# MeryylleA/Lunaris-Orion

Hardware: AMD Instinct MI355X
Metric: 128x128 sprites/sec, VAE training step (train_hybrid.py _process_batch), latent_dim=512 (higher is better)
Workload: dtype f16; 1 GPU; VAE-only training step (fwd+MSE/KL+bwd+clip+AdamW), per-GPU batch 64, latent_dim 512, teacher scalar 0 (--reward_scale 0 --quality_weight 0; the full hybrid step of BASELINE config 3 is the config3_full_hybrid object of a --full run at N=1), gradient_accumulation_steps 1, fp16 MFMA operands / fp32 accumulate, fp32 master weights; global_batch=64, latent_dim=512, parallelism=single, linear_weight_gradients=factored (never materialised)

## Files before the change

### include/lunaris_hip.h

```cpp
#ifndef LUNARIS_HIP_H
#define LUNARIS_HIP_H
#include <stddef.h>
#include <stdint.h>
#ifdef __cplusplus
extern "C" {
#endif

const char* lo_last_error(void);
int lo_version(void);

void lo_prof_enable(int on);
int lo_prof_count(void);
int lo_prof_get(int i, char* name, int name_cap, double* ms, double* flops, double* bytes);

enum {
  LO_KIND_CONV3_S1 = 0,
  LO_KIND_CONV3_S2 = 1,
  LO_KIND_CONVT4_S2 = 2,
  LO_KIND_CONV3_S1_DGRAD = 3,
  LO_KIND_CONV3_S2_DGRAD = 4,
  LO_KIND_CONVT4_S2_DGRAD = 5,
  LO_KIND_LINEAR = 6
};


size_t lo_packed_weight_elems_for(int kind, int B, int H, int W, int Cin, int Cout);
int lo_pack_weight_for(int kind, int B, int H, int W, int Cin, int Cout, const float* w, void* wp, void* stream);
int lo_conv_forward(int kind, int B, int H, int W, int Cin, int Cout, const void* in, const void* wp, const float* bias,
                    const void* add_src, void* out, float* gn_partial, int* mt_out, void* stream);
int lo_quantize_act_f8(const void* x16, void* x8, size_t n, void* stream);
int lo_pack_weight_f8_for(int kind, int B, int H, int W, int Cin, int Cout, const void* wp16, void* wp8, float* wscale, void* stream);
int lo_conv_forward_f8(int kind, int B, int H, int W, int Cin, int Cout, const void* in8, const void* wp8, const float* wscale,
                       const float* bias, const void* add_src, void* out, float* gn_partial, int* mt_out, void* stream);
int lo_conv3x3_fused_tap_forward(int B, int H, int W, int Cin, int Cout, int fp8, const void* in, const void* wp, const float* wscale,
                                 const float* bias, int leaky_relu, void* out, float* bn_partial, void* stream);
int lo_teacher_conv3x3_forward_f8(int B, int H, int W, int Cin, int Cout, const void* in8, const void* wp8, const float* wscale,
                                  const float* bias, int leaky_relu, void* out, float* bn_partial, int* rows_out, void* stream);
int lo_linear_splitk(int M, int K, int N, const void* x, const void* wp, const float* bias, float* slab, int nsplit,
                     float* out32, void* out16, void* stream);
size_t lo_wgrad_slab_bytes_for(int kind, int B, int H, int W, int Cin, int Cout);
int lo_conv_wgrad(int kind, int B, int H, int W, int Cin, int Cout, const void* x, const void* dy, float* slab,
                  float* grad, float scale, void* stream);

int lo_gn_mish_forward(const void* v, const float* gn_partial, int MT, const float* gamma, const float* beta,
                       const void* other, void* y, float* stats, int B, int HW, int C, int mode, void* stream);
int lo_gn_nchunk_for(int HW, int C);
int lo_gn_mish_backward(const void* dy, const void* v, const void* other, const float* stats, const float* gamma,
                        const float* beta, void* ds, void* dv, float* P1, float* P2, float* dgamma, float* dbeta,
                        float* dbias, int B, int HW, int C, int mode, float scale, void* stream);

int lo_first_conv_forward(const float* x, const float* w, const float* bias, void* v, float* gn_partial, int B, void* stream);
int lo_first_conv_wgrad_op(const float* x, const void* dv, float* partial , float* dw, int B, float scale, void* stream);
int lo_image_dgrad_op(const void* dy, int cout, int stride, const float* w, int B, float scale, float* dx, void* stream);
int lo_final_conv_forward(const void* a4, const float* w, const float* bias, const float* target, float* recon,
                          float* mse_partial, int B, void* stream);
int lo_final_conv_backward(const void* a4, const float* w, const float* recon, const float* target, const float* drecon,
                           const float* coef_dev, float gscale, void* da4, float* partial , float* dw,
                           float* db, int B, float scale, void* stream);

int lo_decode_sprites_u8(const void* u8_hwc, float* out_chw, int B, void* stream);

int lo_selfattn2d_forward(const float* x, const float* wq, const float* bq, const float* wk, const float* bk, const float* wv,
                          const float* bv, const float* gamma, float* q, float* k, float* v, float* out, int B, int C,
                          int N, void* stream);
size_t lo_selfattn2d_backward_scratch_elems(int B, int C, int N);
int lo_selfattn2d_backward(const float* x, const float* wq, const float* wk, const float* wv, const float* gamma,
                           const float* q, const float* k, const float* v, const float* dy, float* scratch, float* dx,
                           float* dwq, float* dbq, float* dwk, float* dbk, float* dwv, float* dbv, float* dgamma, int B,
                           int C, int N, void* stream);

int lo_clip_adamw_step(float* p, const float* g, float* m, float* v, size_t n, float max_norm, float lr, float beta1,
                       float beta2, float eps, float weight_decay, int step, float* scratch, void* stream);

int lo_clip_adamw_step_presummed(float* p, const float* g, float* m, float* v, size_t n, size_t presummed_begin, float max_norm,
                                 float lr, float beta1, float beta2, float eps, float weight_decay, int step, float* scratch,
                                 void* stream);

typedef struct LoVae LoVae;
int lo_vae_create(int batch, int latent_dim, LoVae** out);
#define LO_VAE_FP8_FWD 1u
int lo_vae_create_ex(int batch, int latent_dim, unsigned flags, LoVae** out);
void lo_vae_destroy(LoVae* h);
int lo_vae_set_gradnorm_scratch(LoVae* h, float* scratch);
int lo_gradnorm_early_range(const float* flat_grads, size_t begin, size_t end, float* scratch, void* stream);
int lo_vae_set_async_handover(LoVae* h, int on);
int lo_vae_wait_handover(LoVae* h, void* stream);
int lo_vae_gradnorm_presummed(const LoVae* h);
int lo_vae_num_params(const LoVae* h);
// ... 111 lines not shown
```

### lunaris_orion_amd/_lib.py

```python
from __future__ import annotations

import ctypes as C
import os

import torch

HERE = os.path.dirname(os.path.abspath(__file__))
LIB_PATH = os.path.join(HERE, "liblunaris_hip.so")

if not os.path.exists(LIB_PATH):
    raise ImportError(
        f"{LIB_PATH} not found: build it with `python -m lunaris_orion_amd.build` (hipcc, gfx950). "
        "There is no CPU or PyTorch fallback for the lunaris_orion_amd hot path."
    )

lib = C.CDLL(LIB_PATH, mode=C.RTLD_GLOBAL)

vp, f32p, i32, sz, u64, flt = C.c_void_p, C.c_void_p, C.c_int, C.c_size_t, C.c_uint64, C.c_float

SIGNATURES = {
    "lo_last_error": (C.c_char_p, []),
    "lo_version": (i32, []),
    "lo_prof_enable": (None, [i32]),
    "lo_prof_count": (i32, []),
    "lo_prof_get": (i32, [i32, C.c_char_p, i32, C.POINTER(C.c_double), C.POINTER(C.c_double), C.POINTER(C.c_double)]),
    "lo_packed_weight_elems_for": (sz, [i32] * 6),
    "lo_pack_weight_for": (i32, [i32] * 6 + [f32p, vp, vp]),
    "lo_conv_forward": (i32, [i32] * 6 + [vp, vp, f32p, vp, vp, f32p, C.POINTER(C.c_int), vp]),
    "lo_quantize_act_f8": (i32, [vp, vp, sz, vp]),
    "lo_pack_weight_f8_for": (i32, [i32] * 6 + [vp, vp, f32p, vp]),
    "lo_conv_forward_f8": (i32, [i32] * 6 + [vp, vp, f32p, f32p, vp, vp, f32p, C.POINTER(C.c_int), vp]),
    "lo_conv3x3_fused_tap_forward": (i32, [i32] * 6 + [vp, vp, f32p, f32p, i32, vp, f32p, vp]),
    "lo_teacher_conv3x3_forward_f8": (i32, [i32] * 5 + [vp, vp, f32p, f32p, i32, vp, f32p, C.POINTER(C.c_int), vp]),
    "lo_linear_splitk": (i32, [i32, i32, i32, vp, vp, f32p, f32p, i32, f32p, vp, vp]),
    "lo_wgrad_slab_bytes_for": (sz, [i32] * 6),
    "lo_conv_wgrad": (i32, [i32] * 6 + [vp, vp, f32p, f32p, flt, vp]),
    "lo_gn_mish_forward": (i32, [vp, f32p, i32, f32p, f32p, vp, vp, f32p, i32, i32, i32, i32, vp]),
    "lo_gn_nchunk_for": (i32, [i32, i32]),
    "lo_gn_mish_backward": (i32, [vp, vp, vp, f32p, f32p, f32p, vp, vp, f32p, f32p, f32p, f32p, f32p, i32, i32, i32, i32, flt, vp]),
    "lo_first_conv_forward": (i32, [f32p, f32p, f32p, vp, f32p, i32, vp]),
    "lo_first_conv_wgrad_op": (i32, [f32p, vp, f32p, f32p, i32, flt, vp]),
    "lo_image_dgrad_op": (i32, [vp, i32, i32, f32p, i32, flt, f32p, vp]),
    "lo_final_conv_forward": (i32, [vp, f32p, f32p, f32p, f32p, f32p, i32, vp]),
    "lo_final_conv_backward": (i32, [vp, f32p, f32p, f32p, f32p, f32p, flt, vp, f32p, f32p, f32p, i32, flt, vp]),
    "lo_decode_sprites_u8": (i32, [vp, f32p, i32, vp]),
    "lo_selfattn2d_forward": (i32, [f32p] * 12 + [i32, i32, i32, vp]),
    "lo_selfattn2d_backward_scratch_elems": (C.c_size_t, [i32, i32, i32]),
    "lo_selfattn2d_backward": (i32, [f32p] * 18 + [i32, i32, i32, vp]),
    "lo_clip_adamw_step": (i32, [f32p, f32p, f32p, f32p, sz, flt, flt, flt, flt, flt, flt, i32, f32p, vp]),
    "lo_teacher_create": (i32, [i32, i32, i32, i32, C.POINTER(C.c_void_p)]),
    "lo_teacher_create_ex": (i32, [i32, i32, i32, i32, C.c_uint, C.POINTER(C.c_void_p)]),
    "lo_teacher_destroy": (None, [vp]),
    "lo_teacher_num_tensors": (i32, [vp]),
    "lo_teacher_tensor_name": (C.c_char_p, [vp, i32]),
    "lo_teacher_tensor_numel": (sz, [vp, i32]),
    "lo_teacher_tensor_offset": (C.c_longlong, [vp, i32]),
    "lo_teacher_flat_elems": (sz, [vp]),
    "lo_teacher_workspace_bytes": (sz, [vp]),
    "lo_teacher_pack": (i32, [vp, f32p, vp, vp]),
    "lo_teacher_forward": (i32, [vp, f32p, f32p, vp, i32, flt, u64, f32p, f32p, f32p, f32p, f32p, vp]),
    "lo_teacher_last_path": (i32, [vp]),
    "lo_dropout_mask": (i32, [u64, i32, flt, sz, vp, vp]),
    "lo_teacher_grad_range": (i32, [vp, C.POINTER(C.c_size_t), C.POINTER(C.c_size_t)]),
    "lo_teacher_heads_backward": (i32, [vp, f32p, vp, f32p, flt, f32p, f32p, vp]),
    "lo_teacher_heads_saved": (i32, [vp, C.POINTER(C.c_size_t), C.POINTER(C.c_size_t)]),
    "lo_teacher_full_backward_bytes": (C.c_size_t, [vp]),
    "lo_teacher_full_backward_ex": (i32, [vp, f32p, f32p, vp, vp, f32p, f32p, f32p, f32p, f32p, f32p, flt, u64, flt, f32p, f32p, vp]),
    "lo_teacher_full_backward_dx": (i32, [vp, f32p, f32p, vp, vp, f32p, f32p, f32p, f32p, f32p, f32p, flt, u64, flt, f32p, f32p, f32p, vp]),
    "lo_teacher_forward_keep": (i32, [vp, f32p, f32p, vp, vp, flt, u64, f32p, f32p, f32p, f32p, f32p, vp]),
    "lo_teacher_full_backward": (i32, [vp, f32p, f32p, vp, vp, f32p, flt, flt, f32p, f32p, vp]),
    "lo_teacher_clip_adamw_full": (i32, [vp, f32p, f32p, f32p, f32p, flt, flt, flt, flt, flt, flt, i32, f32p, vp]),
    "lo_teacher_full_param_count": (i32, [vp, C.POINTER(C.c_size_t), C.POINTER(C.c_size_t)]),
    "lo_teacher_heads_backward_ex": (i32, [vp, f32p, f32p, f32p, f32p, f32p, f32p, f32p, flt, u64, f32p, f32p, vp]),
    "lo_hybrid_reward": (i32, [f32p, f32p, i32, flt, flt, flt, flt, flt, f32p, f32p, f32p, vp]),
    "lo_vae_create": (i32, [i32, i32, C.POINTER(C.c_void_p)]),
    "lo_vae_create_ex": (i32, [i32, i32, C.c_uint, C.POINTER(C.c_void_p)]),
# ... 79 lines not shown
```

### lunaris_orion_amd/csrc/lo_api.hip

```cpp
#include "lo_internal.h"
#include "lo_conv.h"
#include "lo_norm.h"
#include "../../include/lunaris_hip.h"
#include <stdio.h>
#include <string.h>
#include <stdlib.h>
#include <vector>


extern "C" const char* lo_last_error(void) { return lo_get_error(); }
extern "C" int lo_version(void) { return 1; }

extern "C" size_t lo_packed_weight_elems_for(int kind, int B, int H, int W, int Cin, int Cout) {
  LoGeom g;
  if (lo_make_geom(&g, kind, B, H, W, Cin, Cout) != LO_OK) return 0;
  return lo_packed_weight_elems(g);
}
extern "C" int lo_pack_weight_for(int kind, int B, int H, int W, int Cin, int Cout, const float* w, void* wp, void* stream) {
  LoGeom g;
  LO_TRY(lo_make_geom(&g, kind, B, H, W, Cin, Cout));
  return lo_pack_weight(w, (f16*)wp, g, S(stream));
}
extern "C" int lo_conv_forward(int kind, int B, int H, int W, int Cin, int Cout, const void* in, const void* wp,
                               const float* bias, const void* add_src, void* out, float* gn_partial, int* mt_out,
// ... 69 lines not shown
  LoGeom g;
  LO_REQUIRE(kind == LO_CONV3_S1 || kind == LO_CONV3_S2 || kind == LO_CONVT4_S2 || kind == LO_LINEAR,
             "lo_conv_wgrad: kind %d is not a forward op", kind);
  LO_TRY(lo_make_geom(&g, kind, B, H, W, Cin, Cout));
  return lo_wgrad_run(g, (const f16*)x, (const f16*)dy, slab, grad, scale, S(stream));
}
extern "C" int lo_gn_mish_forward(const void* v, const float* gn_partial, int MT, const float* gamma, const float* beta,
                                  const void* other, void* y, float* stats, int B, int HW, int C, int mode, void* stream) {
  return lo_gn_forward({(const f16*)v, stats, gamma, beta, B, HW, C},
                       {.partial = gn_partial, .MT = MT, .other = (const f16*)other, .mode = mode, .y = (f16*)y}, S(stream));
}
extern "C" int lo_gn_nchunk_for(int HW, int C) { return lo_gn_nchunk(HW, C); }
extern "C" int lo_gn_mish_backward(const void* dy, const void* v, const void* other, const float* stats, const float* gamma,
                                   const float* beta, void* ds, void* dv, float* P1, float* P2, float* dgamma, float* dbeta,
                                   float* dbias, int B, int HW, int C, int mode, float scale, void* stream) {
  return lo_gn_bwd({(const f16*)v, stats, gamma, beta, B, HW, C},
                   {.dy = (const f16*)dy, .other = (const f16*)other, .mode = mode, .ds = (f16*)ds, .dv = (f16*)dv, .P1 = P1, .P2 = P2},
                   dgamma, dbeta, dbias, scale, S(stream));
}
extern "C" int lo_first_conv_forward(const float* x, const float* w, const float* bias, void* v, float* gn_partial, int B,
                                     void* stream) {
  return lo_first_conv_fwd(x, w, bias, (f16*)v, gn_partial, B, S(stream));
}
extern "C" int lo_first_conv_wgrad_op(const float* x, const void* dv, float* partial, float* dw, int B, float scale, void* stream) {
  return lo_first_conv_wgrad(x, (const f16*)dv, partial, dw, B, scale, S(stream));
}
extern "C" int lo_image_dgrad_op(const void* dy, int cout, int stride, const float* w, int B, float scale, float* dx, void* stream) {
  return lo_image_dgrad((const f16*)dy, cout, stride, w, B, scale, dx, S(stream));
}
extern "C" int lo_final_conv_forward(const void* a4, const float* w, const float* bias, const float* target, float* recon,
                                     float* mse_partial, int B, void* stream) {
  return lo_final_conv_fwd((const f16*)a4, w, bias, target, recon, mse_partial, B, S(stream));
}
extern "C" int lo_final_conv_backward(const void* a4, const float* w, const float* recon, const float* target,
                                      const float* drecon, const float* coef_dev, float gscale, void* da4, float* partial,
                                      float* dw, float* db, int B, float scale, void* stream) {
  return lo_final_conv_bwd((const f16*)a4, w, recon, target, drecon, coef_dev, gscale, (f16*)da4, partial, dw, db, B, scale,
                           S(stream));
}
extern "C" int lo_clip_adamw_step(float* p, const float* g, float* m, float* v, size_t n, float max_norm, float lr,
                                  float beta1, float beta2, float eps, float weight_decay, int step, float* scratch,
                                  void* stream) {
  LO_TRY(lo_gradnorm(g, n, max_norm, scratch, scratch + 1024, S(stream)));
  return lo_adamw(p, g, m, v, n, scratch + 1024, lr, beta1, beta2, eps, weight_decay, step, S(stream));
}

extern "C" int lo_clip_adamw_step_presummed(float* p, const float* g, float* m, float* v, size_t n, size_t presummed_begin, float max_norm,
                                            float lr, float beta1, float beta2, float eps, float weight_decay, int step, float* scratch,
                                            void* stream) {
  LO_REQUIRE(p && g && m && v && scratch && presummed_begin <= n && presummed_begin % 4 == 0, "lo_clip_adamw_step_presummed: bad argument");
  LO_TRY(lo_gradnorm_split(g, presummed_begin, max_norm, scratch, scratch + 1024, S(stream)));
  return lo_adamw(p, g, m, v, n, scratch + 1024, lr, beta1, beta2, eps, weight_decay, step, S(stream));
}

extern "C" int lo_decode_sprites_u8(const void* u8_hwc, float* out_chw, int B, void* stream) {
  LO_REQUIRE(u8_hwc && out_chw && B > 0, "lo_decode_sprites_u8: bad argument");
  return lo_decode_sprites((const uint8_t*)u8_hwc, out_chw, B, S(stream));
}

extern "C" int lo_selfattn2d_forward(const float* x, const float* wq, const float* bq, const float* wk, const float* bk,
                                     const float* wv, const float* bv, const float* gamma, float* q, float* k, float* v,
                                     float* out, int B, int C, int N, void* stream) {
  LO_REQUIRE(x && wq && bq && wk && bk && wv && bv && gamma && q && k && v && out, "lo_selfattn2d_forward: null argument");
  return lo_selfattn2d_fwd(x, wq, bq, wk, bk, wv, bv, gamma, q, k, v, out, B, C, N, S(stream));
}

// ... 43 lines not shown
```

### lunaris_orion_amd/csrc/lo_edge.hip

```cpp
#include "lo_common.h"
#include <stdlib.h>

#define FC_W 128
#define FC_OW 64
#define FC_CO 64

__device__ __forceinline__ void fc_stage_rows(const float* __restrict__ x, float (*xs)[3][FC_W + 2], int n, int oy, int tid) {
  for (int i = tid; i < 3 * 3 * (FC_W + 2); i += 256) {
    int col = i % (FC_W + 2);
    int r = (i / (FC_W + 2)) % 3;
    int ci = i / (3 * (FC_W + 2));
    int iy = 2 * oy - 1 + r, ix = col - 1;
    float v = 0.f;
    if ((unsigned)iy < 128u && (unsigned)ix < 128u) v = x[(((size_t)n * 3 + ci) * 128 + iy) * 128 + ix];
    xs[ci][r][col] = v;
  }
}

template <int ROWS>
__global__ __launch_bounds__(256) void lo_first_conv_fwd_mfma_kernel(const float* __restrict__ x, const float* __restrict__ w,
                                                                     const float* __restrict__ bias, f16* __restrict__ v,
                                                                     float* __restrict__ gn_partial) {
  constexpr int NR = 2 * ROWS + 1, RP = FC_W + 2;
  __shared__ float xs[3][NR][RP];
// ... 249 lines not shown
    const int py = wave * 4 + rr;
    f32x4 acc = {0.f, 0.f, 0.f, 0.f};
#pragma unroll
    for (int t = 0; t < 9; ++t) {
      const int r = t / 3, sx = t % 3;
      const f16x8 af = *reinterpret_cast<const f16x8*>(tile + ((py + r) * LC_TP + m + sx) * LC_PITCH + g * 16);
      acc = __builtin_amdgcn_mfma_f32_16x16x32_f16(af, wb[t], acc, 0, 0, 0);
    }
    f32x4 lo;
#pragma unroll
    for (int j = 0; j < 4; ++j) lo[j] = __shfl_down(acc[j], 3, 64);
    if (m < 3) {
      const int oy = ty * LC_T + py, ox = tx * LC_T + 4 * g;
      const size_t o = (((size_t)n * 3 + m) * 128 + oy) * 128 + ox;
      f32x4 rv;
#pragma unroll
      for (int j = 0; j < 4; ++j) rv[j] = lc_tanh(acc[j] + lo[j] + bv);
      *reinterpret_cast<f32x4*>(recon + o) = rv;
      if (mse_partial) {
        const f32x4 tv = *reinterpret_cast<const f32x4*>(target + o);
#pragma unroll
        for (int j = 0; j < 4; ++j) { const float d = rv[j] - tv[j]; sq += d * d; }
      }
    }
  }
  if (mse_partial) {
    const float e = lo_wave_sum(sq);
    if (lane == 0) red[wave] = e;
    __syncthreads();
    if (tid == 0) mse_partial[((size_t)n * gridDim.y + ty) * gridDim.x + tx] = red[0] + red[1] + red[2] + red[3];
  }
}

struct LcBwdArgs {
  const f16* a4;
  const float* w;
  const float* recon;
  const float* target;
  const float* drecon;
  const float* coef;
  float gscale;
  f16* da4;
  float* partial;
};

__device__ __attribute__((aligned(256))) unsigned int lo_zero_page_e[64];
static_assert(sizeof(lo_zero_page_e) >= 1 * 16, "lc_dma_a4: 16 B per lane, all lanes at offset 0 of the zero page");
static_assert(sizeof(lo_zero_page_e) >= 64 * 4, "lc_dma_rt: 64 lanes x 4 B, lane-linear in the zero page");
#define LC_PATCH_BYTES (21 * 1024)
__device__ __forceinline__ void lc_dma_a4(const f16* __restrict__ a4, unsigned int lds_base, int n, int ty, int tx, int wave, int lane) {
  const unsigned char* zpage = reinterpret_cast<const unsigned char*>(lo_zero_page_e);
#pragma unroll
  for (int i = 0; i < 6; ++i) {
    const int k = wave + 4 * i;
    if (k >= 21) break;
    const int q = k * 64 + lane, p = q >> 2, slot = q & 3;
    const int y = p / LC_TP, xx = p - y * LC_TP;
    const int iy = ty * LC_T - 1 + y, ix = tx * LC_T - 1 + xx;
    const void* src = zpage;
    if (p < LC_TP * LC_TP && (unsigned)iy < 128u && (unsigned)ix < 128u) src = a4 + (((size_t)n * 128 + iy) * 128 + ix) * LC_CI + slot * 8;
    lo_dma16(src, __builtin_amdgcn_readfirstlane(lds_base + k * 1024));
  }
}
__device__ __forceinline__ void lo_dma4(const void* gptr, unsigned int lds_off) {
  asm volatile("s_mov_b32 m0, %1\n\ts_nop 0\n\tglobal_load_lds_dword %0, off" ::"v"(gptr), "s"(lds_off) : "memory");
}
// ... 150 lines not shown
    const int k = i / 32, ci = i % 32;
    const int rs = k / 3, co = k % 3;
    outp[(size_t)co * 288 + ci * 9 + rs] = t;
  }
  if (tid < 3) outp[864 + tid] = bred[0][tid] + bred[1][tid] + bred[2][tid] + bred[3][tid];
}

int lo_first_conv_fwd(const float* x, const float* w, const float* bias, f16* v, float* gn_partial, int B, hipStream_t st) {
  LoProfScope _p("lo_first_conv_fwd", 2.0 * B * 4096 * 64 * 27, (double)B * (3 * 16384 * 4 + 4096 * 64 * 2), st);
  hipLaunchKernelGGL((lo_first_conv_fwd_mfma_kernel<4>), dim3(16, B), dim3(256), 0, st, x, w, bias, v, gn_partial);
  LO_LAUNCH_CHECK("first_conv_fwd");
  return LO_OK;
}
int lo_first_conv_wgrad(const float* x, const f16* dv, float* partial, float* dw, int B, float scale, hipStream_t st) {
  LoProfScope _p("lo_first_conv_wgrad(+sum)", 2.0 * B * 4096 * 64 * 27, (double)B * (3 * 16384 * 4 + 4096 * 64 * 2), st);
  hipLaunchKernelGGL((lo_first_conv_wgrad_mfma_kernel<4>), dim3(16, B), dim3(256), 0, st, x, dv, partial);
  LO_LAUNCH_CHECK("first_conv_wgrad");
  hipLaunchKernelGGL(lo_colsum_kernel, dim3((1728 + 15) / 16), dim3(256), 0, st, partial, dw, B * 16, 1728, 1728, scale);
  LO_LAUNCH_CHECK("first_conv_wgrad_sum");
  return LO_OK;
}
int lo_colsum(const float* partial, float* out, int nrow, int ncol, int stride, float scale, hipStream_t st) {
  hipLaunchKernelGGL(lo_colsum_kernel, dim3((ncol + 15) / 16), dim3(256), 0, st, partial, out, nrow, ncol, stride, scale);
  LO_LAUNCH_CHECK("colsum");
  return LO_OK;
}
int lo_final_conv_fwd(const f16* a4, const float* w, const float* bias, const float* target, float* recon,
                      float* mse_partial, int B, hipStream_t st) {
  LoProfScope _p("lo_final_conv_fwd", 2.0 * B * 16384 * 3 * 288, (double)B * 16384 * (32 * 2 + 3 * 4 * 2), st);
  hipLaunchKernelGGL(lo_final_conv_fwd_mfma_kernel, dim3(8, 8, B), dim3(256), 0, st, a4, w, bias, target, recon, mse_partial);
  LO_LAUNCH_CHECK("final_conv_fwd");
  return LO_OK;
}
int lo_final_conv_bwd(const f16* a4, const float* w, const float* recon, const float* target, const float* drecon,
                      const float* coef, float gscale, f16* da4, float* partial, float* dw, float* db, int B, float scale,
                      hipStream_t st, hipStream_t sum_st, hipEvent_t sum_after) {
  LcBwdArgs a{a4, w, recon, target, drecon, coef, gscale, da4, partial};
  LoProfScope _p("lo_final_conv_bwd(+sums)", 4.0 * B * 16384 * 3 * 288, (double)B * 16384 * (32 * 2 * 2 + 3 * 4 * 2), st);
  constexpr int rows = 8;
  LO_LAUNCH_STOP(lo_final_conv_bwd_kernel<8>, dim3(rows, B), dim3(256), 0, st, a);
  LO_LAUNCH_CHECK("final_conv_bwd");
  if (sum_st && sum_after) { LO_HIP(hipStreamWaitEvent(sum_st, sum_after, 0)); st = sum_st; }
  hipLaunchKernelGGL(lo_colsum_kernel, dim3((864 + 15) / 16), dim3(256), 0, st, partial, dw, B * rows, 864, 867, scale);
  LO_LAUNCH_CHECK("final_conv_dw");
  hipLaunchKernelGGL(lo_colsum_kernel, dim3(1), dim3(256), 0, st, partial + 864, db, B * rows, 3, 867, scale);
  LO_LAUNCH_CHECK("final_conv_db");
  return LO_OK;
}
```

### lunaris_orion_amd/csrc/lo_internal.h

```cpp
#pragma once
#include "lo_common.h"

static inline hipStream_t S(void* s) { return reinterpret_cast<hipStream_t>(s); }
#define LO_TRY(call)            \
  do {                          \
    int _r = (call);            \
    if (_r != LO_OK) return _r; \
  } while (0)

const char* lo_get_error();

int lo_first_conv_fwd(const float* x, const float* w, const float* bias, f16* v, float* gn_partial, int B, hipStream_t st);
int lo_first_conv_wgrad(const float* x, const f16* dv, float* partial, float* dw, int B, float scale, hipStream_t st);
int lo_colsum(const float* partial, float* out, int nrow, int ncol, int stride, float scale, hipStream_t st);

int lo_image_dgrad(const f16* dy, int cout, int stride, const float* w, int B, float scale, float* dx, hipStream_t st);
int lo_final_conv_fwd(const f16* a4, const float* w, const float* bias, const float* target, float* recon,
                      float* mse_partial, int B, hipStream_t st);
int lo_final_conv_bwd(const f16* a4, const float* w, const float* recon, const float* target, const float* drecon,
                      const float* coef, float gscale, f16* da4, float* partial, float* dw, float* db, int B, float scale,
                      hipStream_t st, hipStream_t sum_st = nullptr, hipEvent_t sum_after = nullptr);

int lo_head_reduce(const float* slab, const float* bias, const float* eps_in, uint64_t seed, float* mu, float* logvar,
                   f16* z, float* eps_out, float* kl_partial, int B, int L, int nsplit, hipStream_t st, float* mu_user = nullptr,
                   float* logvar_user = nullptr);
int lo_loss_finalize(const float* mse_partial, int n_mse, const float* kl_partial, int n_kl, float rw, float kw, float adv,
                     const float* adv_dev, float accum, float ls, float* losses, float* coefs, float n_rec, float n_lat,
                     hipStream_t st);
int lo_latent_bwd(const f16* dz, const float* mu, const float* logvar, const float* eps, const float* coefs,
                  const float* gmu, const float* glv, float gscale, f16* dml, int B, int L, hipStream_t st);
int lo_colsum_f16(const f16* x, float* out, int M, int N, float scale, hipStream_t st);
int lo_cast_f32_f16(const float* src, f16* dst, size_t n, hipStream_t st);
int lo_scale_f32(float* x, size_t n, float scale, hipStream_t st);
int lo_dp_pack_f16_run(const float* g, f16* wire, size_t n, float scale, hipStream_t st);
int lo_dp_unpack_f16_run(const f16* wire, float* g, size_t n, float inv_scale, hipStream_t st);
int lo_dp_unpack_f16_sumsq_run(const f16* wire, float* g, size_t n, float inv_scale, float* scratch, hipStream_t st);
int lo_dp_sum_shares_run(const void* recv, void* share, int world, size_t chunk, int is_f16, float inv_world, hipStream_t st);
int lo_transpose_cast(const float* src, f16* dst, int R, int C, hipStream_t st);
int lo_gradnorm(const float* g, size_t n, float max_norm, float* partial, float* norm_out, hipStream_t st,
                const unsigned int* fail = nullptr);
int lo_sumsq_range(const float* g, size_t begin, size_t end, float* partial, hipStream_t st);
int lo_gradnorm_split(const float* g, size_t presummed_begin, float max_norm, float* partial, float* norm_out, hipStream_t st,
                      const unsigned int* fail = nullptr);
int lo_grad_scale_pick_run(const float* const g[5], const size_t n[5], float* scratch, hipStream_t st);
int lo_scale_copy_dev_run(const float* src, float* dst, size_t n, const float* scale_dev, hipStream_t st);
int lo_scale_dev_run(float* x, size_t n, const float* scale_dev, const unsigned int* fail, hipStream_t st);
int lo_adamw(float* p, const float* g, float* m, float* v, size_t n, const float* norm, float lr, float beta1, float beta2,
             float eps, float wd, int step, hipStream_t st, f16* cast = nullptr);

int lo_selfattn2d_fwd(const float* x, const float* wq, const float* bq, const float* wk, const float* bk, const float* wv,
                      const float* bv, const float* gamma, float* q, float* k, float* v, float* out, int B, int C, int N,
// ... 20 lines not shown
```

### lunaris_orion_amd/csrc/lo_vae.h

```cpp
#pragma once
#include "lo_internal.h"
#include "lo_conv.h"
#include "lo_norm.h"
#include "../../include/lunaris_hip.h"
#include <stdio.h>
#include <string.h>
#include <stdlib.h>
#include <vector>

#define WSP(T, off) reinterpret_cast<T*>(reinterpret_cast<unsigned char*>(ws) + (off))
#define PRM(i) (P + h->p_off[(i)])
#define GRD(i) (G + h->p_off[(i)])

struct ConvLayer {
  int kind = 0;
  int H = 0, W = 0, Cin = 0, Cout = 0;
  int Ho = 0, Wo = 0;
  LoGeom gf{}, gd{};
  int p_w = 0, p_b = 0, p_gw = 0, p_gb = 0;
  size_t o_wp_f = 0, o_wp_d = 0;
  size_t o_v = 0, o_a = 0;
  size_t o_part = 0, o_stats = 0;
  size_t o_P1 = 0, o_P2 = 0;
  int prow_cap = 0, np1 = 0, np2 = 0;
// ... 24 lines not shown
  int head_split = 32, dfcd_split = 32;
  size_t o_wp_head = 0, o_wp_head_t = 0, o_wp_dfc = 0, o_wp_dfc_t = 0;
  size_t o_xflat = 0, o_slab_head = 0, o_eps = 0, o_z = 0, o_klp = 0, o_mu = 0, o_lv = 0, o_yfc = 0, o_h0 = 0;
  size_t o_msep = 0, o_losses = 0, o_coefs = 0;
  size_t o_G[6] = {}, o_skipg[3] = {}, o_P1 = 0, o_P2 = 0, o_wslab = 0, o_wslab_lin = 0, o_fcw_part = 0, o_lc_part = 0, o_dz = 0, o_dml = 0,
         o_slab_dz = 0, o_gfc = 0;
  size_t o_packjobs = 0;
  std::vector<LoPackJob> packjobs_host;
  int n_packjobs = 0, pack_blocks = 0;
  int n_packjobs_enc = 0, pack_blocks_enc = 0;
  const void* packjobs_for_ws = nullptr;
  const void* packjobs_for_params = nullptr;
  size_t ws_bytes = 0;
  int idx_fc_mu_w = 0, idx_fc_mu_b = 0, idx_fc_lv_w = 0, idx_fc_lv_b = 0, idx_dfc_w = 0, idx_dfc_b = 0, idx_final_w = 0, idx_final_b = 0;
  bool forward_done = false, loss_done = false;
  bool enc_done = false, dec_done = false;
  int dec_skips = 0;
  hipStream_t side = nullptr;
  hipEvent_t ev_dv[4] = {}, ev_join = nullptr, ev_pre = nullptr, ev_range = nullptr;
  bool async_handover = false, range_pending = false;
  hipEvent_t ev_lvl[6] = {};
  bool lvl_pending[6] = {};
  struct { bool pending = false; float* P; const float* G; float* M; float* V; void* ws; const float* norm; float lr, beta1, beta2, eps, wd; int step; } defer;
  int n_packjobs_s4 = 0, pack_blocks_s4 = 0, n_packjobs8_s4 = 0, pack_blocks8_s4 = 0;
  int bwd_layer = 0;
  size_t o_skslab = 0;
  bool gn_local = true;
  int nevent = 0;
  bool overlap = false;
  float* norm_scratch = nullptr;
  bool fuse_gnb = true;
  bool fuse_gnf = false;
  bool fuse_gna = true;
  size_t o_sync_fail = 0;
  bool lin_factored = false, fac_ready = false;
  bool lin_factored_dp = false;
  int Bp = 0;
  size_t o_fac_dmlT = 0, o_fac_xT = 0, o_fac_gfcT = 0, o_fac_zT = 0, o_gram = 0;
  float fac_scale = 1.f;
  int n_cu = 0;
  const void* sync_for_ws = nullptr;
  bool fp8_fwd = false;
  size_t o_eout8[4] = {}, o_h08 = 0, o_packjobs8 = 0;
  std::vector<LoPackF8Job> packjobs8_host;
  int n_packjobs8 = 0, pack_blocks8 = 0;
  int n_packjobs8_enc = 0, pack_blocks8_enc = 0;
};

template <typename H, typename F>
static inline void for_each_layer(H* h, F&& fn) {
  for (int s = 0; s < 4; ++s)
    for (int k = 0; k < 3; ++k) fn(h->enc[s][k]);
  for (int s = 0; s < 4; ++s) fn(h->dec[s]);
}

static inline LoGnLayer vae_gn_layer(const LoVae* h, const ConvLayer& c, const float* P, void* ws) {
  return {WSP(f16, c.o_v), WSP(float, c.o_stats), PRM(c.p_gw), PRM(c.p_gb), h->B, c.Ho * c.Wo, c.Cout};
}
static inline int vae_record_rows(ConvLayer& c, LoGnRows r) {
  LO_REQUIRE(r.p1 <= c.prow_cap && r.p2 <= c.prow_cap, "GroupNorm backward %dx%dx%d: %d / %d rows of P1 / P2 per sample, room for %d",
             c.Ho, c.Wo, c.Cout, r.p1, r.p2, c.prow_cap);
  if (r.p1 > 0) c.np1 = r.p1;
  if (r.p2 > 0) c.np2 = r.p2;
  return LO_OK;
}

// ... 39 lines not shown
```

### lunaris_orion_amd/csrc/lo_vae_plan.hip

```cpp
#include "lo_vae.h"
#include <memory>

namespace {
struct Arena {
  size_t off = 0;
  size_t take(size_t bytes) {
    size_t o = off;
    off += (bytes + 255) & ~(size_t)255;
    return o;
  }
};
bool env_is_zero(const char* v) { return v && atoi(v) == 0; }
const int kEncCh[5] = {3, 64, 128, 256, 512};
const int kDecCh[5] = {512, 256, 128, 64, 32};
}

static int setup_conv_layer(ConvLayer& c, int kind, int B, int H, int W, int Cin, int Cout, int p_w, Arena& ar, bool first) {
  c.kind = kind; c.H = H; c.W = W; c.Cin = Cin; c.Cout = Cout;
  c.p_w = p_w; c.p_b = p_w + 1; c.p_gw = p_w + 2; c.p_gb = p_w + 3;
  if (!first) {
    LO_TRY(lo_make_geom(&c.gf, kind, B, H, W, Cin, Cout));
    int dk = kind == LO_CONV3_S1 ? LO_CONV3_S1_DGRAD : (kind == LO_CONV3_S2 ? LO_CONV3_S2_DGRAD : LO_CONVT4_S2_DGRAD);
    c.Ho = c.gf.Hout; c.Wo = c.gf.Wout;
    LO_TRY(lo_make_geom(&c.gd, dk, B, c.Ho, c.Wo, Cout, Cin));
// ... 139 lines not shown
    for_each_layer(h, [&](ConvLayer& c) {
      if (&c == &h->enc[0][0]) return;
      c.sk_fwd = lo_conv_splitk_plan(c.gf);
      c.sk_dgrad = lo_conv_splitk_plan(c.gd);
      const size_t bf = (size_t)c.sk_fwd * B * c.gf.GH * c.gf.GW * c.gf.Cout * 4, bd = (size_t)c.sk_dgrad * B * c.gd.GH * c.gd.GW * c.gd.Cout * 4;
      slab = bf > slab ? bf : slab;
      slab = bd > slab ? bd : slab;
    });
  h->o_skslab = ar.take(slab > 0 ? slab : 256);
  if (!h->fp8_fwd) return;
  auto enable = [&](ConvLayer& c, size_t* producer_copy) {
    if (lo_conv_choose(c.gf, {.bias = true, .gn_partial = true, .f8 = true}).kernel == LO_CK_NONE) return;
    if (lo_conv_choose(c.gf, {.bias = true, .gn_partial = true}).kernel == LO_CK_CONVT4_PATCH) return;
    c.f8 = true;
    c.o_wp8 = ar.take(lo_packed_weight_elems(c.gf));
    c.o_wscale = ar.take((size_t)c.gf.n_phase * c.Cout * 4);
    if (!*producer_copy) *producer_copy = ar.take((size_t)B * c.H * c.W * c.Cin);
  };
  for (int s = 0; s < 4; ++s) {
    if (s > 0) enable(h->enc[s][0], &h->o_eout8[s - 1]);
    enable(h->enc[s][1], &h->enc[s][0].o_a8);
    enable(h->enc[s][2], &h->enc[s][1].o_a8);
  }
  enable(h->dec[0], &h->o_h08);
  for (int s = 1; s < 4; ++s) enable(h->dec[s], &h->dec[s - 1].o_a8);
  h->o_packjobs8 = ar.take(sizeof(LoPackF8Job) * 32);
}

static void plan_gn_fusions(LoVae* h) {
  h->fuse_gnb = !env_is_zero(getenv("LO_GNB_FUSE"));
  h->gn_local = !env_is_zero(getenv("LO_GN_LOCAL"));
  h->fuse_gnf = getenv("LO_GN_FUSE") && atoi(getenv("LO_GN_FUSE")) != 0 && !h->fp8_fwd;
  h->fuse_gna = h->fuse_gnb && !env_is_zero(getenv("LO_GNB_APPLY_FUSE"));
  int dev = 0, ncu = 0;
  if (hipGetDevice(&dev) == hipSuccess && hipDeviceGetAttribute(&ncu, hipDeviceAttributeMultiprocessorCount, dev) == hipSuccess) h->n_cu = ncu;
  else (void)hipGetLastError();
  if (h->n_cu < 256) h->fuse_gnf = false;
  for_each_layer(h, [&](ConvLayer& c) {
    if (!h->fuse_gnf || &c == &h->enc[0][0] || c.sk_fwd) return;
    const LoConvChoice ch = lo_conv_choose(c.gf, {.bias = true, .gf = true});
    c.gnf = ch.gn_fuse; c.gnf_mts = ch.mts; c.gnf_nt = ch.nt;
  });
}

static void create_side_stream(LoVae* h) {
  h->overlap = getenv("LO_NO_OVERLAP") == nullptr;
  if (!h->overlap) return;
  int prio_least = 0, prio_greatest = 0;
  bool ok;
  if (hipDeviceGetStreamPriorityRange(&prio_least, &prio_greatest) == hipSuccess && prio_least != prio_greatest)
    ok = hipStreamCreateWithPriority(&h->side, hipStreamNonBlocking, prio_least) == hipSuccess;
  else
    ok = hipStreamCreateWithFlags(&h->side, hipStreamNonBlocking) == hipSuccess;
  constexpr unsigned evf = hipEventDisableTiming | hipEventDisableSystemFence;
  for (int i = 0; i < 4 && ok; ++i)
    ok = hipEventCreateWithFlags(&h->ev_dv[i], evf) == hipSuccess;
  ok = ok && hipEventCreateWithFlags(&h->ev_range, hipEventDisableTiming) == hipSuccess;
  ok = ok && hipEventCreateWithFlags(&h->ev_join, evf) == hipSuccess &&
       hipEventCreateWithFlags(&h->ev_pre, evf) == hipSuccess;
  for (int l = 1; l < 6 && ok; ++l) ok = hipEventCreateWithFlags(&h->ev_lvl[l], evf) == hipSuccess;
  if (!ok) { (void)hipGetLastError(); h->overlap = false; }
}

extern "C" int lo_vae_create(int B, int L, LoVae** out) { return lo_vae_create_ex(B, L, 0u, out); }

extern "C" int lo_vae_create_ex(int B, int L, unsigned flags, LoVae** out) {
// ... 135 lines not shown
```

### lunaris_orion_amd/csrc/lo_vae_step.hip

```cpp
#include "lo_vae.h"

static int vae_ensure_sync_init(LoVae* h, void* ws, hipStream_t st) {
  if (h->sync_for_ws == ws) return LO_OK;
  hipError_t e = hipSuccess;
  for_each_layer(h, [&](ConvLayer& c) {
    if (e == hipSuccess) e = hipMemsetAsync(WSP(void, c.o_xcnt), 0, (size_t)h->B * 4, st);
    if (e == hipSuccess) e = hipMemsetAsync(WSP(void, c.o_bcnt), 0, (size_t)h->B * 8 * 4, st);
    c.gnf_epoch = 0; c.gba_epoch = 0;
  });
  LO_HIP(e);
  LO_HIP(hipMemsetAsync(WSP(void, h->o_sync_fail), 0, 256, st));
  h->sync_for_ws = ws;
  return LO_OK;
}

static int conv_gn(LoVae* h, ConvLayer& c, const f16* in, const f16* other, f16* y, int mode, const float* P, void* ws,
                   hipStream_t st, size_t o_in8 = 0, size_t o_y8 = 0) {
  LoProfTag tag("fwd kind%d %dx%d %d->%d", c.kind, c.Ho, c.Wo, c.gf.Cin, c.gf.Cout);
  if (c.sk_fwd && !c.f8 && !o_y8) {
    LO_TRY(lo_conv_run(c.gf, {.in = in, .w = WSP(f16, c.o_wp_f), .slab = WSP(float, h->o_skslab), .nsplit = c.sk_fwd}, st));
    tag.end();
    return lo_gn_forward(vae_gn_layer(h, c, P, ws),
                         {.slab = WSP(float, h->o_skslab), .nsplit = c.sk_fwd, .bias = PRM(c.p_b), .other = other, .mode = mode, .y = y}, st);
  }
  const bool fuse = c.gnf && !c.f8 && !o_y8;
  LoGnFuse gf;
  if (fuse) {
    memset(&gf, 0, sizeof(gf));
    gf.xbuf = WSP(float, c.o_xbuf); gf.counter = WSP(unsigned int, c.o_xcnt);
    gf.MTs = c.gnf_mts; gf.NT = c.gnf_nt;
    gf.target = (++c.gnf_epoch) * (unsigned)(c.gnf_mts * c.gnf_nt);
    gf.gamma = PRM(c.p_gw); gf.beta = PRM(c.p_gb); gf.other = other; gf.y = y; gf.stats = WSP(float, c.o_stats); gf.mode = mode;
    gf.fail = WSP(unsigned int, h->o_sync_fail);
  }
  int r_;
  if (c.f8) {
    LO_REQUIRE(o_in8, "fp8 mode: no e4m3 copy of the input of a conv %d->%d", c.Cin, c.Cout);
    r_ = lo_conv_run_f8(c.gf, WSP(uint8_t, o_in8), WSP(uint8_t, c.o_wp8), WSP(float, c.o_wscale),
                        {.bias = PRM(c.p_b), .out = WSP(f16, c.o_v), .gn_partial = WSP(float, c.o_part)}, st);
  } else {
    r_ = lo_conv_run(c.gf, {.in = in, .w = WSP(f16, c.o_wp_f), .bias = PRM(c.p_b), .out = WSP(f16, c.o_v),
                            .gn_partial = fuse ? nullptr : WSP(float, c.o_part), .gf = fuse ? &gf : nullptr}, st);
  }
  tag.end();
  if (r_ != LO_OK) { if (fuse) --c.gnf_epoch; return r_; }
  if (fuse) return LO_OK;
  return lo_gn_forward(vae_gn_layer(h, c, P, ws), {.partial = WSP(float, c.o_part), .MT = c.MT, .other = other, .mode = mode, .y = y,
                                                   .y8 = o_y8 ? WSP(uint8_t, o_y8) : nullptr}, st);
}

static int vae_decoder_forward(LoVae* h, const f16* const skips[3], const float* P, void* ws, float* recon, const float* target,
                               hipStream_t st) {
  const int B = h->B;
  LO_TRY(vae_ensure_sync_init(h, ws, st));
  LO_TRY(vae_wait_level(h, st, 4));
  LO_TRY(lo_conv_run(h->g_dfc, {.in = WSP(f16, h->o_z), .w = WSP(f16, h->o_wp_dfc), .bias = PRM(h->idx_dfc_b), .out = WSP(f16, h->o_yfc)}, st));
  LO_TRY(lo_nchw_to_nhwc_f16(WSP(f16, h->o_yfc), WSP(f16, h->o_h0), B, 64, 512, st, h->o_h08 ? WSP(uint8_t, h->o_h08) : nullptr));
  const f16* cur = WSP(f16, h->o_h0);
  size_t cur8 = h->o_h08;
  for (int s = 0; s < 4; ++s) {
    ConvLayer& c = h->dec[s];
    const f16* skip = s < 3 ? skips[2 - s] : nullptr;
    LO_TRY(conv_gn(h, c, cur, skip, WSP(f16, c.o_a), skip ? 1 : 0, P, ws, st, cur8, c.o_a8));
    cur = WSP(f16, c.o_a);
    cur8 = c.o_a8;
  }
  h->dec_done = true;
  h->dec_skips = (skips[0] ? 1 : 0) + (skips[1] ? 1 : 0) + (skips[2] ? 1 : 0);
  return lo_final_conv_fwd(cur, PRM(h->idx_final_w), PRM(h->idx_final_b), target, recon, target ? WSP(float, h->o_msep) : nullptr,
                           B, st);
}

static int vae_encoder_forward(LoVae* h, const float* x, const float* eps, uint64_t seed, const float* P, void* ws, float* mu,
                               float* logvar, hipStream_t st);

extern "C" int lo_vae_forward(LoVae* h, const float* x, const float* eps, uint64_t seed, const float* P, void* ws,
                              float* recon, float* mu, float* logvar, const float* target, void* stream) {
  LO_REQUIRE(h && x && P && ws && recon && mu && logvar, "lo_vae_forward: null argument");
  hipStream_t st = S(stream);
  LO_TRY(vae_encoder_forward(h, x, eps, seed, P, ws, mu, logvar, st));
  const f16* skips[3] = {WSP(f16, h->o_eout[0]), WSP(f16, h->o_eout[1]), WSP(f16, h->o_eout[2])};
  LO_TRY(vae_decoder_forward(h, skips, P, ws, recon, target, st));
  h->forward_done = true;
  h->loss_done = false;
  return LO_OK;
}

static int vae_encoder_forward(LoVae* h, const float* x, const float* eps, uint64_t seed, const float* P, void* ws, float* mu,
                               float* logvar, hipStream_t st) {
  const int B = h->B, L = h->L;
  LO_TRY(vae_ensure_sync_init(h, ws, st));
  const f16* cur = nullptr;
  size_t cur8 = 0;
  for (int s = 0; s < 4; ++s) {
    ConvLayer& c0 = h->enc[s][0];
    ConvLayer& c1 = h->enc[s][1];
    ConvLayer& c2 = h->enc[s][2];
    if (s == 0) {
      LO_TRY(lo_first_conv_fwd(x, PRM(c0.p_w), PRM(c0.p_b), WSP(f16, c0.o_v), WSP(float, c0.o_part), B, st));
      LO_TRY(lo_gn_forward(vae_gn_layer(h, c0, P, ws), {.partial = WSP(float, c0.o_part), .MT = c0.MT, .y = WSP(f16, c0.o_a),
                                                        .y8 = c0.o_a8 ? WSP(uint8_t, c0.o_a8) : nullptr}, st));
      LO_TRY(vae_wait_level(h, st, 1));
    } else {
// ... 432 lines not shown
```

Baseline: 24260 sprites/s.

## Fold last decoder GroupNorm+Mish into final conv/tanh/MSE forward kernel

Adds a kernel that computes GroupNorm statistics from conv partials, applies GN+Mish to the last decoder activation, writes the activation for backward, and runs the 3x3 output conv with tanh and MSE partials, all in one pass. The separate GN-apply kernel and its re-read of the activation are skipped, which removes one launch and one full read/write of a 128x128x32 tensor. On by default via the LO_EDGE_FOLD env flag when the layer is not fp8, split-K, or GN-fused. It adds a halo-ring shared-memory scheme and hi/lo fp16 weight split, and correctness depends on the halo and stats handling.

```diff
diff --git a/include/lunaris_hip.h b/include/lunaris_hip.h
--- a/include/lunaris_hip.h
+++ b/include/lunaris_hip.h
@@ -54,6 +54,9 @@
 int lo_image_dgrad_op(const void* dy, int cout, int stride, const float* w, int B, float scale, float* dx, void* stream);
 int lo_final_conv_forward(const void* a4, const float* w, const float* bias, const float* target, float* recon,
                           float* mse_partial, int B, void* stream);
+int lo_gn_final_conv_forward(const void* v, const float* gn_partial, int MT, const float* gamma, const float* beta,
+                             const float* w, const float* bias, const float* target, void* a4, float* stats, float* recon,
+                             float* mse_partial, int B, void* stream);
 int lo_final_conv_backward(const void* a4, const float* w, const float* recon, const float* target, const float* drecon,
                            const float* coef_dev, float gscale, void* da4, float* partial , float* dw,
                            float* db, int B, float scale, void* stream);
diff --git a/lunaris_orion_amd/_lib.py b/lunaris_orion_amd/_lib.py
--- a/lunaris_orion_amd/_lib.py
+++ b/lunaris_orion_amd/_lib.py
@@ -42,6 +42,7 @@
     "lo_first_conv_wgrad_op": (i32, [f32p, vp, f32p, f32p, i32, flt, vp]),
     "lo_image_dgrad_op": (i32, [vp, i32, i32, f32p, i32, flt, f32p, vp]),
     "lo_final_conv_forward": (i32, [vp, f32p, f32p, f32p, f32p, f32p, i32, vp]),
+    "lo_gn_final_conv_forward": (i32, [vp, f32p, i32, f32p, f32p, f32p, f32p, f32p, vp, f32p, f32p, f32p, i32, vp]),
     "lo_final_conv_backward": (i32, [vp, f32p, f32p, f32p, f32p, f32p, flt, vp, f32p, f32p, f32p, i32, flt, vp]),
     "lo_decode_sprites_u8": (i32, [vp, f32p, i32, vp]),
     "lo_selfattn2d_forward": (i32, [f32p] * 12 + [i32, i32, i32, vp]),
diff --git a/lunaris_orion_amd/csrc/lo_api.hip b/lunaris_orion_amd/csrc/lo_api.hip
--- a/lunaris_orion_amd/csrc/lo_api.hip
+++ b/lunaris_orion_amd/csrc/lo_api.hip
@@ -125,6 +125,12 @@
                                      float* mse_partial, int B, void* stream) {
   return lo_final_conv_fwd((const f16*)a4, w, bias, target, recon, mse_partial, B, S(stream));
 }
+extern "C" int lo_gn_final_conv_forward(const void* v, const float* gn_partial, int MT, const float* gamma, const float* beta,
+                                        const float* w, const float* bias, const float* target, void* a4, float* stats,
+                                        float* recon, float* mse_partial, int B, void* stream) {
+  return lo_gn_final_conv_fwd((const f16*)v, gn_partial, MT, gamma, beta, w, bias, target, (f16*)a4, stats, recon, mse_partial, B,
+                              S(stream));
+}
 extern "C" int lo_final_conv_backward(const void* a4, const float* w, const float* recon, const float* target,
                                       const float* drecon, const float* coef_dev, float gscale, void* da4, float* partial,
                                       float* dw, float* db, int B, float scale, void* stream) {
diff --git a/lunaris_orion_amd/csrc/lo_edge.hip b/lunaris_orion_amd/csrc/lo_edge.hip
--- a/lunaris_orion_amd/csrc/lo_edge.hip
+++ b/lunaris_orion_amd/csrc/lo_edge.hip
@@ -305,6 +305,172 @@
   }
 }
 
+#define GF_SW 32
+#define GF_R 8
+#define GF_RING 10
+#define GF_PW (GF_SW + 2)
+struct GfArgs {
+  const f16* v; const float* partial; int MT; const float* gamma; const float* beta;
+  const float* w; const float* bias; const float* target;
+  f16* a4; float* stats; float* recon; float* mse_partial;
+};
+__global__ __launch_bounds__(256, 4) void lo_gn_final_conv_fwd_kernel(GfArgs a) {
+  __shared__ __attribute__((aligned(16))) unsigned char ring[GF_RING * GF_PW * LC_PITCH];
+  __shared__ __attribute__((aligned(16))) f16 wf[9 * 4 * 8 * 8];
+  __shared__ float s_stat[16];
+  __shared__ __attribute__((aligned(16))) float s_ss[4][16];
+  __shared__ __attribute__((aligned(16))) float tgs[3][GF_R][GF_SW];
+  __shared__ float red[4];
+  const int tid = threadIdx.x, lane = tid & 63, m = lane & 15, g = lane >> 4;
+  const int wave = __builtin_amdgcn_readfirstlane(tid >> 6);
+  const int n = blockIdx.y, x0 = (blockIdx.x & 3) * GF_SW, y0 = (blockIdx.x >> 2) * 32;
+  const int ch = tid & 3, px = (tid >> 2) & 31, rh = tid >> 7;
+  const int hr = lane >> 3, hcol = (lane >> 2) & 1 ? GF_SW + 1 : 0;
+  const int hx = x0 - 1 + hcol;
+  const bool hin = (unsigned)hx < 128u;
+  const f16* vn = a.v + (size_t)n * (16384 * LC_CI);
+  f16* an = a.a4 + (size_t)n * (16384 * LC_CI);
+  const int oi = (x0 + px) * LC_CI + ch * 8;
+  const int oh = (hin ? hx : x0) * LC_CI + ch * 8;
+  unsigned char* ri = ring + (px + 1) * LC_PITCH + ch * 16;
+  unsigned char* rhp = ring + hcol * LC_PITCH + ch * 16;
+  const f16x8 zero8 = {0, 0, 0, 0, 0, 0, 0, 0};
+  auto rowc = [&](int j) __attribute__((always_inline)) { const int iy = y0 - 1 + j; return iy < 0 ? 0 : iy > 127 ? 127 : iy; };
+  auto load_i = [&](int j) __attribute__((always_inline)) {
+    return *reinterpret_cast<const f16x8*>(vn + oi + rowc(j) * (128 * LC_CI));
+  };
+  auto load_h = [&](int j) __attribute__((always_inline)) {
+    return *reinterpret_cast<const f16x8*>(vn + oh + rowc(j) * (128 * LC_CI));
+  };
+  auto keep = [&](f16x8 y, bool in) __attribute__((always_inline)) {
+    const unsigned int msk = in ? 0xffffffffu : 0u;
+    u32x4 b = __builtin_bit_cast(u32x4, y);
+    b[0] &= msk; b[1] &= msk; b[2] &= msk; b[3] &= msk;
+    return __builtin_bit_cast(f16x8, b);
+  };
+  f16x8 p0 = load_i(rh), ph, cur[4], curh;
+  if (wave == 3 && hr < 2) ph = load_h(hr);
+#pragma unroll
+  for (int k = 0; k < 4; ++k) cur[k] = load_i(2 + rh + 2 * k);
+  if (wave == 0) curh = load_h(2 + hr);
+  const float gm = a.gamma[tid & 31], bt = a.beta[tid & 31];
+  for (int i = tid; i < 3 * LC_CI * 9; i += 256) {
+    const int t = i % 9, ci = (i / 9) % LC_CI, co = i / (9 * LC_CI);
+    const float wv = a.w[i];
+    const f16 hi = (f16)wv;
+    const int slot = ((t * 4 + (ci >> 3)) * 8 + co) * 8 + (ci & 7);
+    wf[slot] = hi;
+    wf[slot + 24] = (f16)(wv - (float)hi);
+  }
+  for (int i = tid; i < 9 * 4 * 16; i += 256) wf[(i >> 4) * 64 + 48 + (i & 15)] = (f16)0.f;
+  const float bv = m < 3 ? a.bias[m] : 0.f;
+  lo_gn_group_stats(a.partial, a.MT, n, 1.0f / (16384.0f * 4.0f), s_stat, tid);
+  __syncthreads();
+  if (blockIdx.x == 0 && tid < 16) a.stats[n * 16 + tid] = s_stat[tid];
+  if (tid < 32) {
+    float sc1, sh1;
+    lo_gn_scale_shift(gm, bt, s_stat[(tid >> 2) * 2], s_stat[(tid >> 2) * 2 + 1], sc1, sh1);
+    s_ss[tid >> 3][tid & 7] = sc1;
+    s_ss[tid >> 3][8 + (tid & 7)] = sh1;
+  }
+  __syncthreads();
+  float sc[8], sh[8];
+  auto load_ss = [&]() __attribute__((always_inline)) {
+#pragma unroll
+    for (int q = 0; q < 2; ++q) {
+      const f32x4 c4 = *reinterpret_cast<const f32x4*>(&s_ss[ch][4 * q]), h4 = *reinterpret_cast<const f32x4*>(&s_ss[ch][8 + 4 * q]);
+#pragma unroll
+      for (int j = 0; j < 4; ++j) { sc[4 * q + j] = c4[j]; sh[4 * q + j] = h4[j]; }
+    }
+  };
+  load_ss();
+  const f16* wl = &wf[(g * 8 + (m < 6 ? m : 6)) * 8];
+  {
+    const int iy = y0 - 1 + rh;
+    const f16x8 y = keep(lo_gn_apply8(p0, sc, sh, 0, p0), iy >= 0);
+    if (rh == 1) *reinterpret_cast<f16x8*>(an + oi + iy * (128 * LC_CI)) = y;
+    *reinterpret_cast<f16x8*>(ri + rh * (GF_PW * LC_PITCH)) = y;
+    if (wave == 3 && hr < 2) {
+      const f16x8 yh = keep(lo_gn_apply8(ph, sc, sh, 0, ph), hin && y0 - 1 + hr >= 0);
+      *reinterpret_cast<f16x8*>(rhp + hr * (GF_PW * LC_PITCH)) = yh;
+    }
+  }
+  const bool do_mse = a.target != nullptr && a.mse_partial != nullptr;
+  float sq = 0.f;
+#pragma unroll
+  for (int s = 0; s < 4; ++s) {
+    const int j0 = 2 + GF_R * s;
+    f32x4 tg;
+    if (do_mse && wave < 3)
+      tg = *reinterpret_cast<const f32x4*>(a.target + (size_t)n * (3 * 16384) + (wave * 128 + y0 + GF_R * s + (lane >> 3)) * 128 + x0 + 4 * (lane & 7));
+    f16x8 nxt[4], nxth;
+    if (s + 1 < 4) {
+#pragma unroll
+      for (int k = 0; k < 4; ++k) nxt[k] = load_i(j0 + GF_R + rh + 2 * k);
+      if (wave == ((s + 1) & 3)) nxth = load_h(j0 + GF_R + hr);
+    }
+    load_ss();
+#pragma unroll
+    for (int k = 0; k < 4; ++k) {
+      const int j = j0 + rh + 2 * k, iy = y0 - 1 + j;
+      const f16x8 y = keep(lo_gn_apply8(cur[k], sc, sh, 0, cur[k]), iy < 128);
+      if (j <= 32) *reinterpret_cast<f16x8*>(an + oi + iy * (128 * LC_CI)) = y;
+      *reinterpret_cast<f16x8*>(ri + (j % GF_RING) * (GF_PW * LC_PITCH)) = y;
+    }
+    if (wave == (s & 3)) {
+      const int j = j0 + hr;
+      const f16x8 yh = keep(lo_gn_apply8(curh, sc, sh, 0, curh), hin && y0 - 1 + j < 128);
+      *reinterpret_cast<f16x8*>(rhp + (j % GF_RING) * (GF_PW * LC_PITCH)) = yh;
+    }
+    if (do_mse && wave < 3) *reinterpret_cast<f32x4*>(&tgs[wave][lane >> 3][4 * (lane & 7)]) = tg;
+    f16x8 wb[9];
+#pragma unroll
+    for (int t = 0; t < 9; ++t) wb[t] = *reinterpret_cast<const f16x8*>(wl + t * 256);
+    asm volatile("s_waitcnt lgkmcnt(0)" ::: "memory");
+    __builtin_amdgcn_s_barrier();
+#pragma unroll
+    for (int i = 0; i < 4; ++i) {
+      const int orow = GF_R * s + 2 * wave + (i >> 1), b = i & 1;
+      f32x4 acc = {0.f, 0.f, 0.f, 0.f};
+#pragma unroll
+      for (int t = 0; t < 9; ++t) {
+        const int r = t / 3, sx = t % 3;
+        const f16x8 af = *reinterpret_cast<const f16x8*>(ring + (((orow + r) % GF_RING) * GF_PW + 16 * b + m + sx) * LC_PITCH + g * 16);
+        acc = __builtin_amdgcn_mfma_f32_16x16x32_f16(af, wb[t], acc, 0, 0, 0);
+      }
+      f32x4 lo;
+#pragma unroll
+      for (int j = 0; j < 4; ++j) lo[j] = __shfl_down(acc[j], 3, 64);
+      if (m < 3) {
+        const int o = (m * 128 + y0 + orow) * 128 + x0 + 16 * b + 4 * g;
+        f32x4 rv;
+#pragma unroll
+        for (int j = 0; j < 4; ++j) rv[j] = lc_tanh(acc[j] + lo[j] + bv);
+        *reinterpret_cast<f32x4*>(a.recon + (size_t)n * (3 * 16384) + o) = rv;
+        if (do_mse) {
+          const f32x4 tv = *reinterpret_cast<const f32x4*>(&tgs[m][2 * wave + (i >> 1)][16 * b + 4 * g]);
+#pragma unroll
+          for (int j = 0; j < 4; ++j) { const float d = rv[j] - tv[j]; sq += d * d; }
+        }
+      }
+      __builtin_amdgcn_sched_barrier(0);
+    }
+    if (s + 1 < 4) {
+      asm volatile("s_waitcnt lgkmcnt(0)" ::: "memory");
+      __builtin_amdgcn_s_barrier();
+#pragma unroll
+      for (int k = 0; k < 4; ++k) cur[k] = nxt[k];
+      curh = nxth;
+    }
+  }
+  if (do_mse) {
+    const float e = lo_wave_sum(sq);
+    if (lane == 0) red[wave] = e;
+    __syncthreads();
+    if (tid < 4) a.mse_partial[(size_t)n * 64 + 16 * tid + blockIdx.x] = tid == 0 ? red[0] + red[1] + red[2] + red[3] : 0.f;
+  }
+}
+
 struct LcBwdArgs {
   const f16* a4;
   const float* w;
@@ -521,6 +687,16 @@
   LO_LAUNCH_CHECK("final_conv_fwd");
   return LO_OK;
 }
+int lo_gn_final_conv_fwd(const f16* v, const float* gn_partial, int MT, const float* gamma, const float* beta, const float* w,
+                         const float* bias, const float* target, f16* a4, float* stats, float* recon, float* mse_partial, int B,
+                         hipStream_t st) {
+  LO_REQUIRE(v && gn_partial && MT > 0 && gamma && beta && w && bias && a4 && stats && recon, "lo_gn_final_conv_fwd: null argument");
+  LoProfScope _p("lo_gn_final_conv_fwd", 0.0, (double)B * 16384 * (32 * 2 * 2 + 3 * 4 * (target ? 2 : 1)), st);
+  GfArgs a{v, gn_partial, MT, gamma, beta, w, bias, target, a4, stats, recon, target ? mse_partial : nullptr};
+  hipLaunchKernelGGL(lo_gn_final_conv_fwd_kernel, dim3(16, B), dim3(256), 0, st, a);
+  LO_LAUNCH_CHECK("gn_final_conv_fwd");
+  return LO_OK;
+}
 int lo_final_conv_bwd(const f16* a4, const float* w, const float* recon, const float* target, const float* drecon,
                       const float* coef, float gscale, f16* da4, float* partial, float* dw, float* db, int B, float scale,
                       hipStream_t st, hipStream_t sum_st, hipEvent_t sum_after) {
diff --git a/lunaris_orion_amd/csrc/lo_internal.h b/lunaris_orion_amd/csrc/lo_internal.h
--- a/lunaris_orion_amd/csrc/lo_internal.h
+++ b/lunaris_orion_amd/csrc/lo_internal.h
@@ -17,6 +17,9 @@
 int lo_image_dgrad(const f16* dy, int cout, int stride, const float* w, int B, float scale, float* dx, hipStream_t st);
 int lo_final_conv_fwd(const f16* a4, const float* w, const float* bias, const float* target, float* recon,
                       float* mse_partial, int B, hipStream_t st);
+int lo_gn_final_conv_fwd(const f16* v, const float* gn_partial, int MT, const float* gamma, const float* beta, const float* w,
+                         const float* bias, const float* target, f16* a4, float* stats, float* recon, float* mse_partial, int B,
+                         hipStream_t st);
 int lo_final_conv_bwd(const f16* a4, const float* w, const float* recon, const float* target, const float* drecon,
                       const float* coef, float gscale, f16* da4, float* partial, float* dw, float* db, int B, float scale,
                       hipStream_t st, hipStream_t sum_st = nullptr, hipEvent_t sum_after = nullptr);
diff --git a/lunaris_orion_amd/csrc/lo_vae.h b/lunaris_orion_amd/csrc/lo_vae.h
--- a/lunaris_orion_amd/csrc/lo_vae.h
+++ b/lunaris_orion_amd/csrc/lo_vae.h
@@ -80,6 +80,7 @@
   bool fuse_gnb = true;
   bool fuse_gnf = false;
   bool fuse_gna = true;
+  int edge_fold = 1;
   size_t o_sync_fail = 0;
   bool lin_factored = false, fac_ready = false;
   bool lin_factored_dp = false;
diff --git a/lunaris_orion_amd/csrc/lo_vae_plan.hip b/lunaris_orion_amd/csrc/lo_vae_plan.hip
--- a/lunaris_orion_amd/csrc/lo_vae_plan.hip
+++ b/lunaris_orion_amd/csrc/lo_vae_plan.hip
@@ -195,6 +195,7 @@
   h->gn_local = !env_is_zero(getenv("LO_GN_LOCAL"));
   h->fuse_gnf = getenv("LO_GN_FUSE") && atoi(getenv("LO_GN_FUSE")) != 0 && !h->fp8_fwd;
   h->fuse_gna = h->fuse_gnb && !env_is_zero(getenv("LO_GNB_APPLY_FUSE"));
+  h->edge_fold = getenv("LO_EDGE_FOLD") ? atoi(getenv("LO_EDGE_FOLD")) & 1 : 1;
   int dev = 0, ncu = 0;
   if (hipGetDevice(&dev) == hipSuccess && hipDeviceGetAttribute(&ncu, hipDeviceAttributeMultiprocessorCount, dev) == hipSuccess) h->n_cu = ncu;
   else (void)hipGetLastError();
diff --git a/lunaris_orion_amd/csrc/lo_vae_step.hip b/lunaris_orion_amd/csrc/lo_vae_step.hip
--- a/lunaris_orion_amd/csrc/lo_vae_step.hip
+++ b/lunaris_orion_amd/csrc/lo_vae_step.hip
@@ -15,7 +15,7 @@
 }
 
 static int conv_gn(LoVae* h, ConvLayer& c, const f16* in, const f16* other, f16* y, int mode, const float* P, void* ws,
-                   hipStream_t st, size_t o_in8 = 0, size_t o_y8 = 0) {
+                   hipStream_t st, size_t o_in8 = 0, size_t o_y8 = 0, bool gn_later = false) {
   LoProfTag tag("fwd kind%d %dx%d %d->%d", c.kind, c.Ho, c.Wo, c.gf.Cin, c.gf.Cout);
   if (c.sk_fwd && !c.f8 && !o_y8) {
     LO_TRY(lo_conv_run(c.gf, {.in = in, .w = WSP(f16, c.o_wp_f), .slab = WSP(float, h->o_skslab), .nsplit = c.sk_fwd}, st));
@@ -44,14 +44,19 @@
   }
   tag.end();
   if (r_ != LO_OK) { if (fuse) --c.gnf_epoch; return r_; }
-  if (fuse) return LO_OK;
+  if (fuse || gn_later) return LO_OK;
   return lo_gn_forward(vae_gn_layer(h, c, P, ws), {.partial = WSP(float, c.o_part), .MT = c.MT, .other = other, .mode = mode, .y = y,
                                                    .y8 = o_y8 ? WSP(uint8_t, o_y8) : nullptr}, st);
 }
 
+static bool vae_fold_output_stage(const LoVae* h) {
+  const ConvLayer& c = h->dec[3];
+  return (h->edge_fold & 1) && !c.gnf && !c.sk_fwd && !c.o_a8;
+}
 static int vae_decoder_forward(LoVae* h, const f16* const skips[3], const float* P, void* ws, float* recon, const float* target,
                                hipStream_t st) {
   const int B = h->B;
+  const bool fold = vae_fold_output_stage(h);
   LO_TRY(vae_ensure_sync_init(h, ws, st));
   LO_TRY(vae_wait_level(h, st, 4));
   LO_TRY(lo_conv_run(h->g_dfc, {.in = WSP(f16, h->o_z), .w = WSP(f16, h->o_wp_dfc), .bias = PRM(h->idx_dfc_b), .out = WSP(f16, h->o_yfc)}, st));
@@ -61,14 +66,19 @@
   for (int s = 0; s < 4; ++s) {
     ConvLayer& c = h->dec[s];
     const f16* skip = s < 3 ? skips[2 - s] : nullptr;
-    LO_TRY(conv_gn(h, c, cur, skip, WSP(f16, c.o_a), skip ? 1 : 0, P, ws, st, cur8, c.o_a8));
+    LO_TRY(conv_gn(h, c, cur, skip, WSP(f16, c.o_a), skip ? 1 : 0, P, ws, st, cur8, c.o_a8, s == 3 && fold));
     cur = WSP(f16, c.o_a);
     cur8 = c.o_a8;
   }
   h->dec_done = true;
   h->dec_skips = (skips[0] ? 1 : 0) + (skips[1] ? 1 : 0) + (skips[2] ? 1 : 0);
-  return lo_final_conv_fwd(cur, PRM(h->idx_final_w), PRM(h->idx_final_b), target, recon, target ? WSP(float, h->o_msep) : nullptr,
-                           B, st);
+  float* msep = target ? WSP(float, h->o_msep) : nullptr;
+  if (fold) {
+    const ConvLayer& c = h->dec[3];
+    return lo_gn_final_conv_fwd(WSP(f16, c.o_v), WSP(float, c.o_part), c.MT, PRM(c.p_gw), PRM(c.p_gb), PRM(h->idx_final_w),
+                                PRM(h->idx_final_b), target, WSP(f16, c.o_a), WSP(float, c.o_stats), recon, msep, B, st);
+  }
+  return lo_final_conv_fwd(cur, PRM(h->idx_final_w), PRM(h->idx_final_b), target, recon, msep, B, st);
 }
 
 static int vae_encoder_forward(LoVae* h, const float* x, const float* eps, uint64_t seed, const float* P, void* ws, float* mu,
```

Measured after the change: 24460 sprites/s, median of 6. No clear change (+0.8%).
